# ThibHlln/smartpy

Hardware: AMD Instinct MI355X
Metric: MC sample-timesteps/sec/GPU; 1e5 LHS x hourly 10-yr forcing (higher is better)
Workload: dtype f64

## Files before the change

smartpy_amd/csrc/smart_device.h:

```cpp
#pragma once

#include "smart_matrix_common.h"

#include <hip/hip_runtime.h>

#include <type_traits>

namespace smart {

constexpr int kMaxDiv = 12;
constexpr int kForcingInsane = 1 << 30;

struct KArgs {
    long N, T, W, gap, R, first_len;
    int report_type;
    int np_mean;
    double dt;
    const double *area;
    const double *forcing;
    const double *params;
    long pstride_c;
    const double *extra;
    const double *initial;
    const double *obs;
// ... 843 lines not shown
            else
                body(k, *p1, 0.0, 0.0, std::true_type{});
        }
        if (pass == 0 && n_groups > 0) {
            const long group = (long)kGroup * gap;
            const double2 *__restrict__ p = f0 + (long)n_lead * gap;
            const_f64 pe = obs + n_lead, pw = dev + n_lead;
            double2 cur[kGroup], nxt[kGroup];
            double e_cur[kGroup] = {}, e_nxt[kGroup] = {}, w_cur[kGroup] = {}, w_nxt[kGroup] = {};
#pragma unroll
            for (int j = 0; j < kGroup; ++j) {
                cur[j] = p[j * gap];
                if constexpr (OBS) {
                    e_cur[j] = pe[j];
                    w_cur[j] = pw[j];
                }
            }
#pragma unroll
            for (int j = 0; j < kGroup; ++j) {
                asm volatile("" ::"s"(cur[j].x), "s"(cur[j].y));
                if constexpr (OBS)
                    asm volatile("" ::"s"(e_cur[j]), "s"(w_cur[j]));
            }
            for (int g = 0; g < n_groups; ++g) {
                if (g + 1 < n_groups) {
                    p += group;
                    if constexpr (OBS) {
                        pe += kGroup;
                        pw += kGroup;
                    }
                }
#pragma unroll
                for (int j = 0; j < kGroup; ++j) {
                    nxt[j] = p[j * gap];
                    if constexpr (OBS) {
                        e_nxt[j] = pe[j];
                        w_nxt[j] = pw[j];
                    }
                }
#pragma unroll
                for (int j = 0; j < kGroup; ++j)
                    body(n_lead + g * kGroup + j, cur[j], e_cur[j], w_cur[j], std::false_type{});
#pragma unroll
                for (int j = 0; j < kGroup; ++j) {
                    cur[j] = nxt[j];
                    e_cur[j] = e_nxt[j];
                    w_cur[j] = w_nxt[j];
                }
            }
        }
    }
}

template <class Body>
__device__ __forceinline__ void interval_loop(const double2 *__restrict__ f, long i0, long i1, long gap, Body &&body)
{
    interval_walk<false>(f, nullptr, nullptr, i0, i1, gap, 0,
                         [&](int k, const double2 v, double, double, auto) { body(k, v); });
}

template <class Body>
__device__ __forceinline__ void interval_loop_obs(const double2 *__restrict__ f, const double *obs, const double *dev,
                                                  long i0, long i1, long gap, int lead, Body &&body)
{
    interval_walk<true>(f, obs + i0, dev + i0, i0, i1, gap, lead, body);
}

constexpr int kPollSleep = 100;
constexpr long kDefaultMaxPolls = 1000000;

struct Work {
    long block, c;
    int seg;
};

__device__ __forceinline__ Work claim_work(const KArgs &a, int sliced_kernel)
{
    Work w;
    if (a.n_seg > 1) {
        unsigned t = 0;
        if (threadIdx.x == 0)
            t = __hip_atomic_fetch_add(reinterpret_cast<unsigned *>(a.hdr) + kHdrTicket + sliced_kernel, 1u,
                                       __ATOMIC_RELAXED, __HIP_MEMORY_SCOPE_AGENT);
        t = (unsigned)__builtin_amdgcn_readfirstlane((int)t);
        const long slot = (long)(t % (unsigned long)a.seg_blocks);
        w.seg = (int)(t / (unsigned long)a.seg_blocks);
        w.c = slot / a.n_blocks;
        w.block = slot % a.n_blocks;
    } else {
        w.block = blockIdx.x;
        w.c = blockIdx.y;
        w.seg = 0;
    }
    return w;
}

__device__ __forceinline__ bool wait_for_slice(const KArgs &a, long slot, int seg)
{
    int *flag = a.seg_flag + slot;
    long polls = 0;
    int v;
    while ((v = __hip_atomic_load(flag, __ATOMIC_RELAXED, __HIP_MEMORY_SCOPE_AGENT)) > -seg && v < seg) {
        __builtin_amdgcn_s_sleep(kPollSleep);
        if (++polls > a.max_polls) {
            raise_status(a, kStatusSliceTimeout);
            return false;
        }
    }
    __builtin_amdgcn_fence(__ATOMIC_ACQUIRE, "agent");
    return v >= seg;
}

__device__ __forceinline__ void publish_slice(const KArgs &a, long slot, int seg, bool good)
{
    asm volatile("s_waitcnt vmcnt(0)" ::: "memory");
    __builtin_amdgcn_fence(__ATOMIC_RELEASE, "agent");
    asm volatile("s_waitcnt vmcnt(0)" ::: "memory");
    if (threadIdx.x == 0)
        __hip_atomic_store(a.seg_flag + slot, good ? seg + 1 : -(seg + 1), __ATOMIC_RELAXED, __HIP_MEMORY_SCOPE_AGENT);
}

constexpr int kReportMean = 0, kReportLast = 1, kReportEvery = 2;

template <class Model, int FORCING, int REPORT = kReportMean>
__device__ __forceinline__ void run_ensemble_merged(const KArgs &a, const double2 *__restrict__ forcing,
                                                    const double *__restrict__ obs_all,
                                                    const double *__restrict__ ws_all, long block, long catchment,
                                                    int seg, int fflags)
{
    constexpr bool piecewise = FORCING != kForcingVarying;
    constexpr bool runs = FORCING == kForcingRuns;
    static_assert(REPORT == kReportMean || (!Model::kSplit && !runs), "raw / every-step reports: merged model, no runs");
    static_assert(REPORT != kReportEvery || !piecewise, "a report every step is a step loop");
    static_assert(Model::kStateFields <= kSegPend, "the model's states end in front of the other hand-over fields");
    const LaneCtx x = lane_ctx(a, block, catchment);
    const long slot = catchment * a.n_blocks + block;
    Model m;
    init_model(a, x, m);
    const long gap = a.gap;
    const long run_len = runs ? run_length(a, fflags) : gap;
    if constexpr (piecewise)
        m.setup_intervals(REPORT == kReportLast ? run_len - 1 : run_len);
    const double2 *__restrict__ f = forcing + x.c * a.T;

    int fits = 0;
    unsigned not_quick = ~0u;
    if constexpr (piecewise && Model::kWetAsm) {
        m.note_capacity();
        const bool fits_b = m.over_mask == 0;
        fits = __builtin_amdgcn_readfirstlane((int)fits_b);
        not_quick = 0u - (unsigned)__builtin_amdgcn_readfirstlane((int)!(fits_b && !(fflags & kForcingInsane)));
        asm("" : "+s"(fits), "+s"(not_quick));
    }
    auto no_bits = [](double x, unsigned unless = 0) {
        unsigned long long b = __builtin_bit_cast(unsigned long long, x) | unless;
        asm("" : "+s"(b));
        return b == 0;
    };
    auto interval = [&](const double2 v, double &acc, double &num, double &den) {
        if constexpr (piecewise && Model::kWetAsm) {
            if (no_bits(v.x, not_quick)) {
                if (no_bits(v.y)) {
                    m.calm_interval(run_len, acc);
                } else {
                    m.dry_interval(-v.y, run_len, acc);
                }
                return;
            }
        }
        const double ex = m.excess(v.x, v.y);
        if (ex < 0.0) {
            m.dry_interval(ex, run_len, acc);
        } else {
            if constexpr (piecewise && Model::kWetAsm)
                m.wet_interval(ex, run_len, acc, num, den, fits);
            else
                m.wet_interval(ex, run_len, acc, num, den);
        }
    };

    [[maybe_unused]] auto interval_last = [&](const double2 v, double &qo, double &qg, double &qi) {
        if constexpr (piecewise && REPORT == kReportLast && Model::kWetAsm) {
            double sink = 0.0, n0 = 0.0, n1 = 0.0;
            if (no_bits(v.x, not_quick)) {
                if (no_bits(v.y)) {
                    m.calm_interval(gap - 1, sink);
                    m.last_step_flows(qo, qg, qi);
                    m.calm_interval(1, sink);
                } else {
                    m.dry_interval_last(-v.y, gap, qo, qg, qi);
                }
                return;
            }
            const double ex = m.excess(v.x, v.y);
            if (ex < 0.0) {
                m.dry_interval_last(ex, gap, qo, qg, qi);
            } else {
                m.wet_interval(ex, gap - 1, sink, n0, n1, fits);
                m.last_step_flows(qo, qg, qi);
                m.wet_interval(ex, 1, sink, n0, n1, fits);
            }
        }
    };

    const long n_warm = a.W / gap, n_all = n_warm + a.R;
    const long g0 = n_all * seg / a.n_seg, g1 = n_all * (seg + 1) / a.n_seg;
    const long wa = g0 < n_warm ? g0 : n_warm, wb = g1 < n_warm ? g1 : n_warm;
    const long ra = g0 > n_warm ? g0 - n_warm : 0, rb = g1 > n_warm ? g1 - n_warm : 0;
    const bool last = seg == a.n_seg - 1;

    Reporter rep;
    rep.init(a, x, obs_all, ws_all);
    [[maybe_unused]] const double *__restrict__ obs_c = obs_all ? obs_all + x.c * a.R : nullptr;
    [[maybe_unused]] const double *__restrict__ dev_c = ws_all ? ws_all + x.c * (kWsHead + a.R) + kWsHead : nullptr;
    [[maybe_unused]] const uint2 *codes_c = a.codes ? a.codes + x.c * code_chunks(a.T) : nullptr;
    [[maybe_unused]] const double2 *f_asm = reinterpret_cast<const double2 *>(a.forcing) + x.c * a.T;
    double num = 0.0, den = 0.0, q_out_total = 0.0;
    [[maybe_unused]] double num_raw = 0.0, den_raw = 0.0;
    double *hand = a.seg_state + (slot * kSegFields) * kWave + x.lane;
    if (seg > 0) {
        if (!wait_for_slice(a, slot, seg)) {
            const double nan = quiet_nan();
            if (a.discharge && x.live)
                for (long r = ra; r < rb; ++r)
                    a.discharge[(x.c * a.R + r) * a.ld + x.n] = nan;
            if (last) {
                if (x.live) {
                    a.gw[x.c * a.N + x.n] = nan;
                    if (a.objfn)
                        for (int i = 0; i < 8; ++i)
                            a.objfn[(x.c * a.N + x.n) * 8 + i] = nan;
                    if (a.final_vars)
                        for (int i = 0; i < 19; ++i)
                            a.final_vars[(x.c * a.N + x.n) * 19 + i] = nan;
                }
            } else {
                publish_slice(a, slot, seg, false);
            }
            return;
        }
        m.load_state(hand, kWave);
        if constexpr (REPORT == kReportLast) {
            num_raw = hand[kSegOutflows * kWave];
            den_raw = hand[kSegDenRaw * kWave];
        } else {
            q_out_total = hand[kSegOutflows * kWave];
        }
        rep.A = hand[kSegA * kWave];
        rep.B = hand[kSegB * kWave];
        rep.C1 = hand[kSegC1 * kWave];
        rep.C2 = hand[kSegC2 * kWave];
        rep.C3 = hand[kSegC3 * kWave];
        rep.shift = hand[kSegShift * kWave];
    }

    double *const park = Model::kSplit ? a.final_vars + (x.c * a.N + x.n) * 19 : nullptr;
    auto park_state = [&]() {
        if constexpr (Model::kSplit) {
            m.save_state(park, 1);
            if constexpr (!piecewise)
                park[15] = m.pend;
        }
    };

    double s0 = 0.0, s1 = 0.0, s2 = 0.0;
    const double inv_gap = 1.0 / (double)gap;
    const bool starts_run = ra == 0 && (rb > 0 || last);
    constexpr bool deferring = !piecewise;
    [[maybe_unused]] const bool first_slice = ra == 0;
    [[maybe_unused]] int store = __builtin_amdgcn_readfirstlane((int)(a.discharge != nullptr));
    asm("" : "+s"(store));
    [[maybe_unused]] const int k_park = Model::kSplit && ra <= a.R - 1 && a.R - 1 < rb ? (int)(a.R - 1 - ra) : -1;
    if constexpr (piecewise)
        rep.begin_rows(a, x, ra);
    if constexpr (runs) {
        const long per = gap / run_len;
        interval_loop(f, wa * per, wb * per, run_len, [&](int, const double2 v) { interval(v, s0, s1, s2); });
        if (starts_run)
            m.begin_run();
        long j = 0, r = ra;
        double acc = 0.0;
        rep.prime(a, ra);
        interval_loop(f, ra * per, rb * per, run_len, [&](int, const double2 v) {
            if (Model::kSplit && j == 0 && r == a.R - 1)
                park_state();
            interval(v, acc, num, den);
            if (++j == per) {
                rep.emit_ahead(a, x, r, acc * inv_gap);
                q_out_total += acc;
                acc = 0.0;
                j = 0;
                ++r;
            }
        });
    } else if constexpr (piecewise && REPORT == kReportLast) {
        interval_loop(f, wa, wb, gap, [&](int, const double2 v) { interval_last(v, s0, s1, s2); });
        if (starts_run)
            m.begin_run();
        if (rep.want_obj) {
            interval_loop_obs(f, rep.obs, rep.ws + kWsHead, ra, rb, gap, first_slice ? 1 : 0,
                              [&](int k, const double2 v, const double e, const double w, auto lead_tag) {
                                  double qo, qg, qi;
                                  interval_last(v, qo, qg, qi);
                                  rep.template emit_interval<true, decltype(lead_tag)::value, false>(
                                      store, a.ld, first_slice && k == 0, qo, e, w);
                                  num_raw += qg;
                                  den_raw += qi;
                              });
        } else {
            interval_loop(f, ra, rb, gap, [&](int, const double2 v) {
                double qo, qg, qi;
                interval_last(v, qo, qg, qi);
                rep.template emit_interval<false, false, true>(store, a.ld, false, qo, 0.0, 0.0);
                num_raw += qg;
                den_raw += qi;
            });
        }
    } else if constexpr (piecewise) {
        interval_loop(f, wa, wb, gap, [&](int, const double2 v) { interval(v, s0, s1, s2); });
        if (starts_run)
            m.begin_run();
        if (rep.want_obj) {
            interval_loop_obs(f, rep.obs, rep.ws + kWsHead, ra, rb, gap, first_slice ? 1 : 0,
                              [&](int k, const double2 v, const double e, const double w, auto lead_tag) {
                                  if (Model::kSplit && k == k_park)
                                      park_state();
                                  double acc = 0.0;
                                  interval(v, acc, num, den);
                                  rep.template emit_interval<true, decltype(lead_tag)::value, false>(
                                      store, a.ld, first_slice && k == 0, acc * inv_gap, e, w);
                                  q_out_total += acc;
                              });
        } else {
            interval_loop(f, ra, rb, gap, [&](int k, const double2 v) {
                if (Model::kSplit && k == k_park)
                    park_state();
                double acc = 0.0;
                interval(v, acc, num, den);
                rep.template emit_interval<false, false, true>(store, a.ld, false, acc * inv_gap, 0.0, 0.0);
                q_out_total += acc;
            });
        }
    } else {
        m.begin_lazy(seg > 0 ? hand[kSegPend * kWave] : 0.0);
        long k = 0, r = ra;
        (void)k;
        double acc = 0.0;
        auto report = [&]() __attribute__((always_inline)) {
            auto emit = [&](const double val) __attribute__((always_inline)) {
                rep.emit(a, x, r, val);
                rep.next_row(a);
            };
            if constexpr (REPORT == kReportMean) {
// ... 244 lines not shown
```

smartpy_amd/csrc/smart_fast_arms.h:

```cpp
#pragma once

#define SMART_A_ALIGN8 ".p2align 3\n\t"
#define SMART_A_ALIGN8_ODD ".p2align 3\n\ts_nop 0\n\t"
#define SMART_A_ROUTE                                                                                                  \
    "v_mul_f64 %[t0], %[cg], %[yg]\n\t"                                                                                \
    "v_fma_f64 %[t0], %[cf], %[yf], %[t0]\n\t"                                                                         \
    "v_fma_f64 %[t0], %[cs], %[ys], %[t0]\n\t"                                                                         \
    "v_add_f64 %[acc], %[acc], %[riv]\n\t"                                                                             \
    "v_fma_f64 %[riv], %[riv], %[oma], %[t0]\n\t"
#define SMART_A_ROUTE_LAST                                                                                             \
    "v_mul_f64 %[qg], %[cg], %[yg]\n\t"                                                                                \
    "v_fma_f64 %[qi], %[cf], %[yf], %[qg]\n\t"                                                                         \
    "v_fma_f64 %[qi], %[cs], %[ys], %[qi]\n\t"                                                                         \
    "v_mov_b64_e64 %[acc], %[riv]\n\t"                                                                                 \
    "v_fma_f64 %[riv], %[riv], %[oma], %[qi]\n\t"
#define SMART_A_CASCADE                                                                                                \
    "v_add_f64 %[l0], %[pend], -%[l0]\n\t"                                                                             \
    "v_mul_f64 %[t0], %[pc], %[l0]\n\t"                                                                                \
    "v_max_f64 %[t0], %[t0], 0\n\t"                                                                                    \
    "v_cmp_lt_f64 vcc, 0, %[t0]\n\t"                                                                                   \
    "s_cbranch_vccz 2f\n\t"                                                                                            \
    "v_add_f64 %[l1], %[t0], -%[l1]\n\t"                                                                               \
    "v_mul_f64 %[t0], %[pc], %[l1]\n\t"                                                                                \
    "v_max_f64 %[t0], %[t0], 0\n\t"                                                                                    \
// ... 320 lines not shown
    "91:\n\t" SMART_P_NINE("0", route, "s[36:37]", "s[38:39]", "s[40:41]", "s[42:43]", SMART_P_TAIL_A0, deep,          \
                           calm_split, zeros, drain, rain_split, dry_split)                                            \
        SMART_P_NINE("1", route, "s[44:45]", "s[46:47]", "s[48:49]", "s[50:51]", tail_b0, deep, calm_split, zeros,     \
                     drain, rain_split, dry_split)                                                                     \
            SMART_P_NINE("2", route, "s[52:53]", "s[54:55]", "s[56:57]", "s[58:59]", SMART_P_TAIL_A1, deep,            \
                         calm_split, zeros, drain, rain_split, dry_split)                                              \
                SMART_P_NINE("3", route, "s[60:61]", "s[62:63]", "s[64:65]", "s[66:67]", SMART_P_TAIL_B1, deep,        \
                             calm_split, zeros, drain, rain_split, dry_split)                                          \
                    SMART_P_QUADS("4", "0", "1", route, "s[38:39]", "s[42:43]", "s[46:47]", "s[50:51]", tail_b0, deep, \
                                  calm_split, dry_split)                                                               \
                        SMART_P_QUADS("4", "2", "3", route, "s[54:55]", "s[58:59]", "s[62:63]", "s[66:67]",            \
                                      SMART_P_TAIL_B1, deep, calm_split, dry_split) ".p2align 3\n\t" block94             \
    "95:\n\t" report SMART_P_NEXT_INTERVAL("s[52:67]", "s[70:71]", "s68") "99:\n\t"
#define SMART_A_PAIRS_STRETCH(route, report, deep, calm_split, zeros, drain, rain_split, dry_split)                    \
    SMART_A_PAIRS_STRETCH_X(route, report, SMART_P_ENTRY_EVEN, SMART_P_TAIL_B0, "", deep, calm_split, zeros, drain,    \
                            rain_split, dry_split)
#define SMART_A_PAIRS_STRETCH_ODD(route, report, deep, calm_split, zeros, drain, rain_split, dry_split)                \
    SMART_A_PAIRS_STRETCH_X(route, report, SMART_P_ENTRY_ODD, SMART_P_TAIL_B0_ODD, SMART_P_REPORT94(report), deep,     \
                            calm_split, zeros, drain, rain_split, dry_split)
#define SMART_P_CLOBBERS                                                                                               \
    "s52", "s53", "s54", "s55", "s56", "s57", "s58", "s59", "s60", "s61", "s62", "s63", "s64", "s65", "s66", "s67",    \
        "s70", "s71", "s72", "s73", "s74", "s76", "s77", "s78", "s79", "vcc", "scc"
#define SMART_S_CLOBBERS                                                                                               \
    "s36", "s37", "s38", "s39", "s40", "s41", "s42", "s43", "s44", "s45", "s46", "s47", "s48", "s49", "s50", "s51",    \
        "s68", "s69", "s75", "s80", "s81", "s82", "s83", "s84", "s85", SMART_P_CLOBBERS

#define SMART_E_STORE "global_store_dwordx2 %[row], %[acc], off" SMART_STORE_MOD "\n\tv_lshl_add_u64 %[row], %[ld], 3, %[row]\n\t"
#define SMART_E_MOMENTS(e, w, whi) SMART_R_MOMENTS("%[acc]", e, w, whi)
#define SMART_E_SUM "v_add_f64 %[qtot], %[qtot], %[acc]\n\t"
#define SMART_E_C_N(rep, id) SMART_P_ARM_C_N(SMART_A_ROUTE_LAST, id, "", "") rep
#define SMART_E_C_Q(rep) SMART_P_ARM_C_Q(SMART_A_ROUTE_LAST, "", "") rep
#define SMART_E_C_F(rep) SMART_P_ARM_C_F(SMART_A_ROUTE_LAST, "", "") rep
#define SMART_E_D(pe, rep) SMART_A_DRY(SMART_A_ROUTE_LAST, pe, "") rep
#define SMART_E_R(rn, pe, id, rep) "s_nop 0\n\t" SMART_P_ARM_R(SMART_A_ROUTE_LAST, rn, pe, id, "", "", "", "") "s_nop 0\n\t" rep
#define SMART_E_R_Q(rn, pe, rep) "s_nop 0\n\t" SMART_P_ARM_R_Q(SMART_A_ROUTE_LAST, rn, pe, "", "", "", "") "s_nop 0\n\t" rep
#define SMART_E_R_F(rn, pe, rep) "s_nop 0\n\t" SMART_P_ARM_R_F(SMART_A_ROUTE_LAST, rn, pe, "", "", "", "") "s_nop 0\n\t" rep
#define SMART_E_BLOCK(pos, k, body) ".org 91b+(" pos "*9+" k ")*" SMART_P_STR(SMART_E_STRIDE) "\n\t" body
#define SMART_E_NINE(pos, rx, px, r0, ry, py, r1, tail)                                                                \
    SMART_E_BLOCK(pos, "0", SMART_E_C_N(r0, "0") SMART_E_C_Q(r1) tail SMART_P_OOL(SMART_A_CASC_CALM_OOL("0")))         \
    SMART_E_BLOCK(pos, "1", SMART_E_C_N(r0, "0") SMART_E_D(py, r1) tail SMART_P_OOL(SMART_A_CASC_CALM_OOL("0")))       \
    SMART_E_BLOCK(pos, "2", SMART_E_C_N(r0, "0") SMART_E_R_Q(ry, py, r1) tail SMART_P_OOL(SMART_A_CASC_CALM_OOL("0"))) \
    SMART_E_BLOCK(pos, "3", SMART_E_D(px, r0) SMART_E_C_F(r1) tail)                                                    \
    SMART_E_BLOCK(pos, "4", SMART_E_D(px, r0) SMART_E_D(py, r1) tail)                                                  \
    SMART_E_BLOCK(pos, "5", SMART_E_D(px, r0) SMART_E_R_F(ry, py, r1) tail)                                            \
    SMART_E_BLOCK(pos, "6", SMART_E_R(rx, px, "0", r0) SMART_E_C_N(r1, "1")                                            \
                                tail SMART_P_OOL(SMART_A_CASC_RAIN_OOL("0")) SMART_P_OOL(SMART_A_CASC_CALM_OOL("1")))  \
    SMART_E_BLOCK(pos, "7", SMART_E_R(rx, px, "0", r0) SMART_E_D(py, r1) tail SMART_P_OOL(SMART_A_CASC_RAIN_OOL("0"))) \
    SMART_E_BLOCK(pos, "8", SMART_E_R(rx, px, "0", r0) SMART_E_R(ry, py, "1", r1)                                      \
                                tail SMART_P_OOL(SMART_A_CASC_RAIN_OOL("0")) SMART_P_OOL(SMART_A_CASC_RAIN_OOL("1")))
#define SMART_E_REQUEST(p, c)                                                                                          \
    "s_add_u32 s73, s73, 64\n\t"                                                                                       \
    "s_load_dwordx16 " p ", %[sp], s73\n\t"                                                                            \
    "s_add_u32 s74, s74, 4\n\t"                                                                                        \
    "s_load_dword " c ", %[cp], s74\n\t"
#define SMART_E_TAIL_P0 "s_waitcnt lgkmcnt(0)\n\t" SMART_E_REQUEST("s[36:51]", "s68") SMART_P_JUMP("s70")
#define SMART_E_TAIL_P1                                                                                                \
    "s_waitcnt lgkmcnt(0)\n\t"                                                                                         \
    "s_add_u32 s72, s72, 1\n\t"                                                                                        \
    "s_cbranch_scc1 99f\n\t" SMART_E_REQUEST("s[52:67]", "s70") SMART_P_JUMP("s68")
#define SMART_E_REP(store, mom, e, w, whi) store mom(e, w, whi) SMART_E_SUM
#define SMART_E_NOMOM(e, w, whi) ""
#define SMART_A_EVERY_STREAM(store, mom)                                                                               \
    "s_getpc_b64 s[78:79]\n\t"                                                                                         \
    "90:\n\t"                                                                                                          \
    "s_add_u32 s78, s78, 91f-90b\n\t"                                                                                  \
    "s_addc_u32 s79, s79, 0\n\t"                                                                                       \
    "s_mov_b32 s77, s79\n\t"                                                                                           \
    "s_load_dwordx16 s[36:51], %[sp], 0x0\n\t"                                                                         \
    "s_load_dword s68, %[cp], 0x0\n\t"                                                                                 \
    "s_mov_b32 s73, 64\n\t"                                                                                            \
    "s_load_dwordx16 s[52:67], %[sp], s73\n\t"                                                                         \
    "s_mov_b32 s74, 4\n\t"                                                                                             \
    "s_load_dword s70, %[cp], s74\n\t"                                                                                 \
    "s_sub_u32 s72, 0, %[quads]\n\t"                                                                                   \
    "s_waitcnt lgkmcnt(0)\n\t" SMART_P_JUMP("s68") ".p2align 6\n\t"                                                    \
    "91:\n\t" SMART_E_NINE("0", "s[36:37]", "s[38:39]", SMART_E_REP(store, mom, "s[40:41]", "s[42:43]", "s43"),        \
                           "s[44:45]", "s[46:47]", SMART_E_REP(store, mom, "s[48:49]", "s[50:51]", "s51"),             \
                           SMART_E_TAIL_P0)                                                                            \
        SMART_E_NINE("1", "s[52:53]", "s[54:55]", SMART_E_REP(store, mom, "s[56:57]", "s[58:59]", "s59"), "s[60:61]",  \
                     "s[62:63]", SMART_E_REP(store, mom, "s[64:65]", "s[66:67]", "s67"), SMART_E_TAIL_P1)              \
            ".p2align 3\n\t"                                                                                           \
            "99:\n\t"
#define SMART_E_CLOBBERS                                                                                               \
    "s36", "s37", "s38", "s39", "s40", "s41", "s42", "s43", "s44", "s45", "s46", "s47", "s48", "s49", "s50", "s51",    \
        "s68", SMART_P_CLOBBERS

#define SMART_G_ARM1(arm, rep) arm rep
#define SMART_G_NINE(pos, v, route, rx, px, r0, ry, py, r1, tail)                                                      \
    SMART_E_BLOCK(pos, v "*9+0", SMART_P_ARM_C_N(route, "0", "", "") r0 SMART_P_ARM_C_Q(route, "", "") r1              \
                                     tail SMART_P_OOL(SMART_A_CASC_CALM_OOL("0")))                                     \
    SMART_E_BLOCK(pos, v "*9+1", SMART_P_ARM_C_N(route, "0", "", "") r0 SMART_A_DRY(route, py, "") r1                  \
                                     tail SMART_P_OOL(SMART_A_CASC_CALM_OOL("0")))                                     \
    SMART_E_BLOCK(pos, v "*9+2", SMART_P_ARM_C_N(route, "0", "", "") r0 "s_nop 0\n\t" SMART_P_ARM_R_Q(                 \
        route, ry, py, "", "", "", "") "s_nop 0\n\t" r1 tail SMART_P_OOL(SMART_A_CASC_CALM_OOL("0")))                  \
    SMART_E_BLOCK(pos, v "*9+3", SMART_A_DRY(route, px, "") r0 SMART_P_ARM_C_F(route, "", "") r1 tail)                 \
    SMART_E_BLOCK(pos, v "*9+4", SMART_A_DRY(route, px, "") r0 SMART_A_DRY(route, py, "") r1 tail)                     \
    SMART_E_BLOCK(pos, v "*9+5", SMART_A_DRY(route, px, "") r0 "s_nop 0\n\t" SMART_P_ARM_R_F(                          \
        route, ry, py, "", "", "", "") "s_nop 0\n\t" r1 tail)                                                          \
    SMART_E_BLOCK(pos, v "*9+6", "s_nop 0\n\t" SMART_P_ARM_R(route, rx, px, "0", "", "", "", "") "s_nop 0\n\t" r0      \
                                     SMART_P_ARM_C_N(route, "1", "", "") r1                                            \
                                         tail SMART_P_OOL(SMART_A_CASC_RAIN_OOL("0"))                                  \
                                             SMART_P_OOL(SMART_A_CASC_CALM_OOL("1")))                                  \
    SMART_E_BLOCK(pos, v "*9+7", "s_nop 0\n\t" SMART_P_ARM_R(route, rx, px, "0", "", "", "", "") "s_nop 0\n\t" r0      \
                                     SMART_A_DRY(route, py, "") r1 tail SMART_P_OOL(SMART_A_CASC_RAIN_OOL("0")))       \
    SMART_E_BLOCK(pos, v "*9+8", "s_nop 0\n\t" SMART_P_ARM_R(route, rx, px, "0", "", "", "", "") "s_nop 0\n\t" r0      \
                                     "s_nop 0\n\t" SMART_P_ARM_R(route, ry, py, "1", "", "", "", "") "s_nop 0\n\t" r1  \
                                         tail SMART_P_OOL(SMART_A_CASC_RAIN_OOL("0"))                                  \
                                             SMART_P_OOL(SMART_A_CASC_RAIN_OOL("1")))
#define SMART_G_REP(value, after, e, w, whi) SMART_P_REPORT_X(value, after, e, w, whi) "s_nop 0\n\t"
#define SMART_G_THREE(pos, route, value, after, rx, px, e0, w0, h0, ry, py, e1, w1, h1, tail)                          \
    SMART_G_NINE(pos, "0", route, rx, px, "", ry, py, "", tail)                                                        \
    SMART_G_NINE(pos, "1", route, rx, px, SMART_G_REP(value, after, e0, w0, h0), ry, py, "", tail)                     \
    SMART_G_NINE(pos, "2", route, rx, px, "", ry, py, SMART_G_REP(value, after, e1, w1, h1), tail)
#define SMART_A_GAP_STREAM(route, value, after)                                                                        \
    "s_getpc_b64 s[78:79]\n\t"                                                                                         \
    "90:\n\t"                                                                                                          \
    "s_add_u32 s78, s78, 91f-90b\n\t"                                                                                  \
    "s_addc_u32 s79, s79, 0\n\t"                                                                                       \
    "s_mov_b32 s77, s79\n\t"                                                                                           \
    "s_load_dwordx16 s[36:51], %[sp], 0x0\n\t"                                                                         \
    "s_load_dword s68, %[cp], 0x0\n\t"                                                                                 \
    "s_mov_b32 s73, 64\n\t"                                                                                            \
    "s_load_dwordx16 s[52:67], %[sp], s73\n\t"                                                                         \
    "s_mov_b32 s74, 4\n\t"                                                                                             \
    "s_load_dword s70, %[cp], s74\n\t"                                                                                 \
    "s_sub_u32 s72, 0, %[quads]\n\t"                                                                                   \
    "s_mov_b32 s85, %[r0]\n\t"                                                                                         \
    "s_waitcnt lgkmcnt(0)\n\t" SMART_P_JUMP("s68") ".p2align 6\n\t"                                                    \
    "91:\n\t" SMART_G_THREE("0", route, value, after, "s[36:37]", "s[38:39]", "s[40:41]", "s[42:43]", "s43",           \
                            "s[44:45]", "s[46:47]", "s[48:49]", "s[50:51]", "s51", SMART_E_TAIL_P0)                    \
        SMART_G_THREE("3", route, value, after, "s[52:53]", "s[54:55]", "s[56:57]", "s[58:59]", "s59", "s[60:61]",     \
                      "s[62:63]", "s[64:65]", "s[66:67]", "s67", SMART_E_TAIL_P1) ".p2align 3\n\t"                     \
                                                                                   "99:\n\t"

#define SMART_A_WET_HEAD SMART_A_ROUTE "v_fma_f64 %[xf], -%[eh], %[tot], %[ex]\n\t" SMART_A_FILL1("l0", "xf")
#define SMART_A_WET_FILL_TAIL                                                                                          \
    SMART_A_FILL1("l1", "t1") SMART_A_FILL1("l2", "t1") SMART_A_FILL1("l3", "t1") SMART_A_FILL1("l4", "t1")            \
        SMART_A_FILL1("l5", "t1") "v_mul_f64 %[xs], %[eh], %[tot]\n\t"                                                 \
                                  "v_fma_f64 %[xf], -%[pd], %[t1], %[xf]\n\t"                                          \
                                  "v_fma_f64 %[xs], %[pd], %[t1], %[xs]\n\t"
#define SMART_A_WET_REST                                                                                               \
    SMART_A_LEAKS_("s1", "p2", "p3", "") "v_add_f64 %[t1], %[tot], -%[ai]\n\t"                                                            \
                    "v_add_f64 %[xf], %[xf], %[t1]\n\t" SMART_A_TOT_XG                                                 \
                    "v_fma_f64 %[ys], %[ys], %[ds], %[xs]\n\t"                                                         \
                    "v_fma_f64 %[yf], %[yf], %[df], %[xf]\n\t"                                                         \
                    "v_fma_f64 %[yg], %[yg], %[dg], %[xg]\n\t"                                                         \
                    "v_add_f64 %[xgs], %[xgs], %[xg]\n\t"
#define SMART_A_WET_STEP SMART_A_WET_HEAD SMART_A_WET_FILL_TAIL SMART_A_WET_REST
#define SMART_A_WET_ABSORBED(fix)                                                                                      \
    SMART_A_WET_HEAD "v_cmp_nle_f64 vcc, %[t1], 0\n\t"                                                                 \
                     "s_cbranch_vccnz " fix "f\n\t"                                                                    \
                     "v_mul_f64 %[xs], %[eh], %[tot]\n\t" SMART_A_WET_REST
#define SMART_A_WET_FULL(fix) SMART_A_WET_HEAD fix ":\n\t" SMART_A_WET_FILL_TAIL SMART_A_WET_REST
#define SMART_A_WET_GROUPS                                                                                             \
    "s_lshr_b32 %[cnt], %[n], 2\n\t"                                                                                  \
    "s_sub_u32 %[cnt], 0, %[cnt]\n\t"                                                                                  \
    "s_cbranch_scc0 9f\n\t"
#define SMART_A_WET_INTERVAL                                                                                           \
    SMART_A_ALIGN8 "s_cmp_eq_u32 %[ok], 0\n\t"                                                                         \
    "s_cbranch_scc1 40f\n\t"                                                                                           \
    "s_and_b32 %[cnt], %[n], 3\n\t"                                                                                  \
    "s_cbranch_scc0 20f\n\t"                                                                                           \
    "s_sub_u32 %[cnt], 0, %[cnt]\n\t"                                                                                  \
    "5:\n\t" SMART_A_WET_ABSORBED("7") "s_add_u32 %[cnt], %[cnt], 1\n\t"                                               \
    "s_cbranch_scc0 5b\n\t"                                                                                            \
    "20:\n\t" SMART_A_WET_GROUPS "25:\n\t" SMART_A_WET_ABSORBED("71") "s_nop 0\n\t" SMART_A_WET_ABSORBED("72")         \
    "s_nop 0\n\t" SMART_A_WET_ABSORBED("73") "s_nop 0\n\t" SMART_A_WET_ABSORBED("74")                        \
    "s_add_u32 %[cnt], %[cnt], 1\n\t"                                                                                  \
    "s_cbranch_scc0 25b\n\t"                                                                                           \
    "s_branch 9f\n\t"                                                                                                  \
    "40:\n\t"                                                                                                          \
    "s_and_b32 %[cnt], %[n], 3\n\t"                                                                                  \
    "s_cbranch_scc0 30f\n\t"                                                                                           \
    "s_sub_u32 %[cnt], 0, %[cnt]\n\t"                                                                                  \
    "6:\n\t" SMART_A_WET_FULL("7") "s_add_u32 %[cnt], %[cnt], 1\n\t"                                                   \
    "s_cbranch_scc0 6b\n\t"                                                                                            \
    "30:\n\t" SMART_A_WET_GROUPS "s_nop 0\n\t"                                                                         \
    "31:\n\t" SMART_A_WET_FULL("71") SMART_A_WET_FULL("72") SMART_A_WET_FULL("73") SMART_A_WET_FULL("74")              \
    "s_add_u32 %[cnt], %[cnt], 1\n\t"                                                                                  \
    "s_cbranch_scc0 31b\n\t"                                                                                           \
    "9:\n\t"
#define SMART_A_CALM_STEP                                                                                              \
    SMART_A_ROUTE SMART_A_LEAKS_("s1", "p2", "p3", "") "v_add_f64 %[xf], %[tot], -%[ai]\n\t" SMART_A_TOT_XG            \
    "v_fma_f64 %[ys], %[ys], %[ds], 0\n\t"                                                                             \
    "v_fma_f64 %[yf], %[yf], %[df], %[xf]\n\t"                                                                         \
    "v_fma_f64 %[yg], %[yg], %[dg], %[xg]\n\t"                                                                         \
    "v_add_f64 %[xgs], %[xgs], %[xg]\n\t"
#define SMART_A_CALM_INTERVAL                                                                                          \
    SMART_A_ALIGN8 "s_add_i32 %[cnt], %[n], 1\n\t"                                                                                    \
    "s_lshr_b32 %[cnt], %[cnt], 1\n\t"                                                                                 \
    "s_bitcmp1_b32 %[n], 0\n\t"                                                                                        \
    "s_cbranch_scc1 6f\n\t"                                                                                            \
    "5:\n\t" SMART_A_CALM_STEP "6:\n\t" SMART_A_CALM_STEP "s_add_i32 %[cnt], %[cnt], -1\n\t"                           \
    "s_cmp_lg_u32 %[cnt], 0\n\t"                                                                                       \
    "s_cbranch_scc1 5b\n\t"
```

smartpy_amd/csrc/smart_fast_model.h:

```cpp
#pragma once

#include "smart_device.h"
#include "smart_fast_arms.h"

namespace smart {

template <bool STIFF, bool GUARD, bool MERGE = false, bool EXITS = true, bool SPLIT = false>
struct FastModel {
    static_assert(!(MERGE && STIFF), "the clamps of structure.py:429-450 act on each reservoir separately");
    static_assert(MERGE || !SPLIT, "SPLIT refines the merged form");
    static constexpr bool kExactDivide = false;
    static constexpr bool kSplit = SPLIT;

    double pT, pC, pD, hz, sz, z;
    double dec_s, dec_f, dec_g, cq_s, cq_f, cq_g;
    double a_r, inv_a_r;
    double a_s, a_f, a_g;
    double car_s, car_f, car_g, om_ar;
    double k_s, k_f, k_g, k_r, mm_to_m3;
    double l0, l1, l2, l3, l4, l5;
    double u_ove, u_dra, u_int, u_sgw, u_dgw, u_riv;
    double q_out, q_in, q_gw;

    __device__ void setup(double area, double dt, const double *p)
// ... 186 lines not shown
    }

    __device__ static void sum_then_fma_in_place(double &sum, double &y, double a, double x)
    {
        asm("v_add_f64 %0, %0, %1\n\tv_fma_f64 %1, %1, %2, %3" : "+v"(sum), "+v"(y) : "v"(a), "v"(x));
    }


    __device__ __forceinline__ void wet_lanes(double ex)
    {
        if (kLeakBalance) {
            double tot = layer_sum();
            wet_balance(ex, ex * hz, tot);
            return;
        }
        const double tot = layer_sum();
        const double hp = hz * tot;
        const double s1 = sz * tot;
        const double of = hp * ex;
        ex = fma(-hp, ex, ex);
        fill(l0, ex, z);
        if (excess_left(ex)) {
            fill(l1, ex, z);
            fill(l2, ex, z);
            fill(l3, ex, z);
            fill(l4, ex, z);
            fill(l5, ex, z);
        }
        const double df = pD * ex;
        double inf = ex - df;
        double sh = 0.0, dp = 0.0;
        const double p2 = s1 * s1, p3 = p2 * s1, p4 = p2 * p2, p5 = p4 * s1, p6 = p3 * p3;
        leak(l0, s1, s1, p6, inf, sh, dp);
        leak(l1, p2, s1 * 0.5, p5, inf, sh, dp);
        leak(l2, p3, s1 * (1.0 / 3.0), p4, inf, sh, dp);
        leak(l3, p4, s1 * 0.25, p3, inf, sh, dp);
        leak(l4, p5, s1 * 0.2, p2, inf, sh, dp);
        leak(l5, p6, s1 * (1.0 / 6.0), s1, inf, sh, dp);
        if (MERGE) {
            const double xg = sh + dp;
            u_ove = fma(u_ove, dec_s, of + df);
            u_int = fma(u_int, dec_f, inf);
            u_sgw = fma(u_sgw, dec_g, xg);
            if (kBalanceSums)
                xg_sum += xg;
        } else {
            u_ove = clamp(fma(u_ove, dec_s, of * cq_s));
            u_dra = clamp(fma(u_dra, dec_s, df * cq_s));
            u_int = clamp(fma(u_int, dec_f, inf * cq_f));
            u_sgw = clamp(fma(u_sgw, dec_g, sh * cq_g));
            u_dgw = clamp(fma(u_dgw, dec_g, dp * cq_g));
        }
    }

    static constexpr bool kLeakBalance = MERGE && !GUARD;
    static_assert(kLeakBalance || !SPLIT, "SPLIT is implemented in wet_balance()");

    static constexpr bool kExits = EXITS;

    __device__ __forceinline__ double deep_leak(double s1, double p2, double p3, double p4, double p5, double p6) const
    {
        return fma(l5, s1, fma(l4, p2, fma(l3, p3, fma(l2, p4, fma(l1, p5, l0 * p6)))));
    }

    __device__ __forceinline__ static double opaque_zero()
    {
        double x;
        asm volatile("v_mov_b64 %0, 0" : "=v"(x));
        return x;
    }

    __device__ static void fill3(double &l, double &ex, double z)
    {
        const double t = l + ex;
        l = fmin(t, z);
        ex = t - l;
    }

    __device__ __forceinline__ void wet_balance(const double ex, const double e_h, double &tot)
    {
        const double s1 = sz * tot;
        const double ex_in = fma(-e_h, tot, ex);
        double rem = ex_in;
        fill3(l0, rem, z);
        if (!kExits || excess_left(rem)) {
            fill3(l1, rem, z);
            if (!kExits || excess_left(rem)) {
                fill3(l2, rem, z);
                fill3(l3, rem, z);
                fill3(l4, rem, z);
                fill3(l5, rem, z);
            }
        }
        const double p2 = s1 * s1, p3 = p2 * s1, p4 = p2 * p2, p5 = p4 * s1, p6 = p3 * p3;
        l0 = fma(-l0, s1, l0);
        l1 = fma(-l1, p2, l1);
        l2 = fma(-l2, p3, l2);
        l3 = fma(-l3, p4, l3);
        l4 = fma(-l4, p5, l4);
        l5 = fma(-l5, p6, l5);
        const double after_int = layer_sum();
        l0 = fma(-l0, s1, l0);
        l1 = fma(-l1, s1 * 0.5, l1);
        l2 = fma(-l2, s1 * (1.0 / 3.0), l2);
        l3 = fma(-l3, s1 * 0.25, l3);
        l4 = fma(-l4, s1 * 0.2, l4);
        l5 = fma(-l5, s1 * (1.0 / 6.0), l5);
        const double deep = SPLIT ? deep_leak(s1, p2, p3, p4, p5, p6) : 0.0;
        l0 = fma(-l0, p6, l0);
        l1 = fma(-l1, p5, l1);
        l2 = fma(-l2, p4, l2);
        l3 = fma(-l3, p3, l3);
        l4 = fma(-l4, p2, l4);
        l5 = fma(-l5, s1, l5);
        const double inf = (tot - after_int) + fma(-pD, rem, ex_in);
        fma_in_place(u_ove, dec_s, fma(pD, rem, e_h * tot));
        fma_in_place(u_int, dec_f, inf);
        const double upper = (l0 + l1) + (l2 + l3), lower = l4 + l5;
        asm("v_add_f64 %0, %1, %2" : "+v"(tot) : "v"(upper), "v"(lower));
        const double xg = after_int - tot;
        fma_in_place(u_sgw, dec_g, xg);
        if (SPLIT) {
            fma_in_place(u_dra, dec_s, pD * rem);
            fma_in_place(u_dgw, dec_g, deep);
        }
        if (kBalanceSums)
            xg_sum += xg;
    }

#ifndef SMART_WET_ASM
#define SMART_WET_ASM 1
#endif
    static constexpr bool kWetAsm = SMART_WET_ASM && kLeakBalance && !kExits && !SPLIT && !STIFF;

    __device__ __forceinline__ void calm_interval(long n, double &acc)
    {
        static_assert(kWetAsm, "calm_interval() is the asm loop of the straight-line merged kernels");
        double tot = layer_sum();
        double t0, t1, xf, xg, w_s1, w_p2, w_p3, w_p4, w_p5, w_p6, w_ai;
        int cnt;
        asm volatile(SMART_A_CALM_INTERVAL
                     : [l0] "+v"(l0), [l1] "+v"(l1), [l2] "+v"(l2), [l3] "+v"(l3), [l4] "+v"(l4), [l5] "+v"(l5),
                       [ys] "+v"(u_ove), [yf] "+v"(u_int), [yg] "+v"(u_sgw), [riv] "+v"(u_riv), [acc] "+v"(acc),
                       [tot] "+v"(tot), [xgs] "+v"(xg_sum), [t0] "=&v"(t0), [t1] "=&v"(t1), [xf] "=&v"(xf),
                       [xg] "=&v"(xg), [s1] "=&v"(w_s1), [p2] "=&v"(w_p2), [p3] "=&v"(w_p3), [p4] "=&v"(w_p4),
                       [p5] "=&v"(w_p5), [p6] "=&v"(w_p6), [ai] "=&v"(w_ai), [cnt] "=&s"(cnt)
                     : [cs] "v"(car_s), [cf] "v"(car_f), [cg] "v"(car_g), [oma] "v"(om_ar), [ds] "v"(dec_s),
                       [df] "v"(dec_f), [dg] "v"(dec_g), [sz] "v"(sz), [k3] "s"(-(1.0 / 3.0)), [k5] "s"(-0.2),
                       [k6] "s"(-(1.0 / 6.0)), [n] "s"((int)n)
                     : "scc");
    }

    __device__ __forceinline__ void wet_interval(double ex, long n, double &acc, double &num, double &den,
                                                 const int fits = 0)
    {
        if constexpr (kWetAsm) {
            const double e_h = ex * hz;
            double tot = layer_sum();
            double t0, t1, xs, xf, xg, w_s1, w_p2, w_p3, w_p4, w_p5, w_p6, w_ai;
            int cnt;
            asm volatile(SMART_A_WET_INTERVAL
                         : [l0] "+v"(l0), [l1] "+v"(l1), [l2] "+v"(l2), [l3] "+v"(l3), [l4] "+v"(l4), [l5] "+v"(l5),
                           [ys] "+v"(u_ove), [yf] "+v"(u_int), [yg] "+v"(u_sgw), [riv] "+v"(u_riv), [acc] "+v"(acc),
                           [tot] "+v"(tot), [xgs] "+v"(xg_sum), [t0] "=&v"(t0), [t1] "=&v"(t1), [xs] "=&v"(xs),
                           [xf] "=&v"(xf), [xg] "=&v"(xg), [s1] "=&v"(w_s1), [p2] "=&v"(w_p2), [p3] "=&v"(w_p3),
                           [p4] "=&v"(w_p4), [p5] "=&v"(w_p5), [p6] "=&v"(w_p6), [ai] "=&v"(w_ai), [cnt] "=&s"(cnt)
                         : [cs] "v"(car_s), [cf] "v"(car_f), [cg] "v"(car_g), [oma] "v"(om_ar), [ds] "v"(dec_s),
                           [df] "v"(dec_f), [dg] "v"(dec_g), [sz] "v"(sz), [z] "v"(z), [pd] "v"(pD), [ex] "v"(ex),
                           [eh] "v"(e_h), [k3] "s"(-(1.0 / 3.0)), [k5] "s"(-0.2), [k6] "s"(-(1.0 / 6.0)),
                           [n] "s"((int)n), [ok] "s"(fits)
                         : "scc", "vcc");
        } else if (kLeakBalance) {
            const double e_h = ex * hz;
            double tot = layer_sum();
#pragma unroll 1
            for (long k = 0; k < n; ++k) {
                route_and_sum(acc, num, den);
                wet_balance(ex, e_h, tot);
            }
        } else {
            for (long k = 0; k < n; ++k) {
                route_and_sum(acc, num, den);
                wet_lanes(ex);
            }
        }
    }

    __device__ __forceinline__ void dry_lanes(double ex)
    {
        double d = -ex;
        dry(l0, d, pC);
        auto handed_down = [](double x) { return GUARD ? x != 0.0 : x > 0.0; };
        if (__builtin_amdgcn_ballot_w64(handed_down(d)) != 0) {
            dry(l1, d, pC);
            if (__builtin_amdgcn_ballot_w64(handed_down(d)) != 0) {
                dry(l2, d, pC);
                dry(l3, d, pC);
                dry(l4, d, pC);
                dry(l5, d, pC);
            }
        }
        u_ove = clamp(u_ove * dec_s);
        u_int = clamp(u_int * dec_f);
        u_sgw = clamp(u_sgw * dec_g);
        if (!MERGE || SPLIT) {
            u_dra = clamp(u_dra * dec_s);
            u_dgw = clamp(u_dgw * dec_g);
        }
    }

    __device__ __forceinline__ void route_and_sum(double &acc, double &num, double &den)
    {
        double q_r = u_riv;
        double u_new;
        if (MERGE && !STIFF && kBalanceSums) {
            q_out = u_riv;
            q_gw = cq_g * u_sgw;
            q_in = fma(cq_s, u_ove, fma(cq_f, u_int, q_gw));
            const double y = fma(car_s, u_ove, fma(car_f, u_int, car_g * u_sgw));
            if (kExits) {
                sum_then_fma_in_place(acc, u_riv, om_ar, y);
            } else {
                acc += u_riv;
                fma_in_place(u_riv, om_ar, y);
            }
            return;
        }
        if (MERGE) {
            u_new = u_riv;
            fma_in_place(u_new, om_ar, fma(car_s, u_ove, fma(car_f, u_int, car_g * u_sgw)));
            q_gw = cq_g * u_sgw;
            q_in = fma(cq_s, u_ove, fma(cq_f, u_int, q_gw));
        } else {
            q_gw = u_sgw + u_dgw;
            q_in = ((u_ove + u_dra) + u_int) + q_gw;
            u_new = fma(q_in - u_riv, a_r, u_riv);
        }
        if (STIFF) {
            if (u_new < 0.0) {
                q_r = 0.95 * fma(u_riv, inv_a_r, q_in);
                u_new = fma(q_in - q_r, a_r, u_riv);
            }
        }
        u_riv = u_new;
        q_out = q_r;
        acc += q_r;
        if (!kBalanceSums) {
            num += q_gw;
            den += q_in;
        }
    }

    static constexpr int kStateFields = 15;

    __device__ void save_state(double *p, int stride) const
    {
        const double v[kStateFields] = {l0, l1, l2, l3, l4, l5, u_ove, u_int, u_sgw, u_riv, g0, r0, xg_sum, u_dra, u_dgw};
#pragma unroll
        for (int i = 0; i < (SPLIT ? 15 : 13); ++i)
            p[i * stride] = v[i];
    }

    __device__ void load_state(const double *p, int stride)
    {
        double v[kStateFields] = {};
#pragma unroll
        for (int i = 0; i < (SPLIT ? 15 : 13); ++i)
            v[i] = p[i * stride];
        l0 = v[0], l1 = v[1], l2 = v[2], l3 = v[3], l4 = v[4], l5 = v[5];
        u_ove = v[6], u_int = v[7], u_sgw = v[8], u_riv = v[9];
        g0 = v[10], r0 = v[11], xg_sum = v[12];
        u_dra = v[13], u_dgw = v[14];
        note_capacity();
    }

    static constexpr bool kBalanceSums = MERGE;
    double g0, r0, xg_sum;

    __device__ void begin_run()
    {
        g0 = u_sgw;
        r0 = u_riv;
        xg_sum = 0.0;
    }

    __device__ void balance_sums(double q_out_total, double &num, double &den) const
    {
        num = cq_g * (xg_sum + (g0 - u_sgw)) / (1.0 - dec_g);
        den = fma(u_riv - r0, inv_a_r, q_out_total);
    }

    __device__ void step(double , double , double ex, double &acc, double &num, double &den)
    {
        if (ex >= 0.0) {
            route_and_sum(acc, num, den);
            wet_lanes(ex);
        } else {
            route_and_sum(acc, num, den);
            dry_lanes(ex);
        }
    }

    __device__ void step(double r, double e, double ex, double &acc, double &num, double &den, StepGeneric)
    {
        step(r, e, ex, acc, num, den);
    }

    __device__ void step(double, double, double ex, double &acc, double &num, double &den, StepAllWet)
    {
        route_and_sum(acc, num, den);
        wet_lanes(ex);
    }

    double pend, tot_c;
    bool zero_ok;
    unsigned long long pend_mask;

    __device__ void begin_lazy(double pending)
    {
        pend = pending;
        pend_mask = __builtin_amdgcn_ballot_w64(pending > 0.0);
        tot_c = layer_sum();
        note_capacity();
// ... 458 lines not shown
```

smartpy_amd/csrc/smart_fast_runs.hip:

```cpp
#include "smart_fast_entry.h"

namespace smart {

SMART_FAST_KERNEL(smart_fast_runs_exits) { merged_kernel<FastModel<false, false, true, true>, kForcingRuns>(a, forcing, obs, ws); }

SMART_FAST_KERNEL(smart_fast_runs) { merged_kernel<FastModel<false, false, true, false>, kForcingRuns>(a, forcing, obs, ws); }

SMART_FAST_KERNEL(smart_fast_runs_states)
{
    merged_kernel<FastModel<false, false, true, true, true>, kForcingRuns>(a, forcing, obs, ws);
}

}
```

Measured before the change: 899.8 billion.

## Run wet intervals under explicit exec mask and reorder divergent dry/calm branches

The wet interval asm now sets the exec mask itself via s_and_saveexec from a ballot of wet lanes, and computes e_h and the layer sum inside the asm. The control flow is reshaped so that the wet, dry and calm paths are taken as separate predicated regions instead of nested branches with an early return, with the aim of cutting divergence overhead. The grouped-by-4 loop now runs before the remainder loop. The main runs kernel also gets a waves_per_eu(2,2) attribute to change register and occupancy tradeoffs. The new structure risks running more paths per interval when lanes mix, and the occupancy pin may cost latency hiding.

```diff
diff --git a/smartpy_amd/csrc/smart_device.h b/smartpy_amd/csrc/smart_device.h
--- a/smartpy_amd/csrc/smart_device.h
+++ b/smartpy_amd/csrc/smart_device.h
@@ -1019,28 +1019,35 @@
         not_quick = 0u - (unsigned)__builtin_amdgcn_readfirstlane((int)!(fits_b && !(fflags & kForcingInsane)));
         asm("" : "+s"(fits), "+s"(not_quick));
     }
-    auto no_bits = [](double x, unsigned unless = 0) {
+    auto bits_of = [](double x, unsigned unless = 0) {
         unsigned long long b = __builtin_bit_cast(unsigned long long, x) | unless;
         asm("" : "+s"(b));
-        return b == 0;
+        return b;
+    };
+    auto same_bits = [](unsigned long long b) {
+        asm("" : "+s"(b));
+        return b;
     };
     auto interval = [&](const double2 v, double &acc, double &num, double &den) {
         if constexpr (piecewise && Model::kWetAsm) {
-            if (no_bits(v.x, not_quick)) {
-                if (no_bits(v.y)) {
+            const unsigned long long rainy = bits_of(v.x, not_quick);
+            if (rainy != 0) {
+                const double ex = m.excess(v.x, v.y);
+                const bool dry = ex < 0.0;
+                m.wet_interval(ex, run_len, acc, num, den, fits, __builtin_amdgcn_ballot_w64(true) & ~__builtin_amdgcn_ballot_w64(dry));
+                if (dry)
+                    m.dry_interval(ex, run_len, acc);
+            }
+            if (same_bits(rainy) == 0) {
+                if (bits_of(v.y) != 0)
+                    m.dry_interval(-v.y, run_len, acc);
+                else
                     m.calm_interval(run_len, acc);
-                } else {
-                    m.dry_interval(-v.y, run_len, acc);
-                }
-                return;
-            }
-        }
-        const double ex = m.excess(v.x, v.y);
-        if (ex < 0.0) {
-            m.dry_interval(ex, run_len, acc);
+            }
         } else {
-            if constexpr (piecewise && Model::kWetAsm)
-                m.wet_interval(ex, run_len, acc, num, den, fits);
+            const double ex = m.excess(v.x, v.y);
+            if (ex < 0.0)
+                m.dry_interval(ex, run_len, acc);
             else
                 m.wet_interval(ex, run_len, acc, num, den);
         }
@@ -1049,23 +1056,25 @@
     [[maybe_unused]] auto interval_last = [&](const double2 v, double &qo, double &qg, double &qi) {
         if constexpr (piecewise && REPORT == kReportLast && Model::kWetAsm) {
             double sink = 0.0, n0 = 0.0, n1 = 0.0;
-            if (no_bits(v.x, not_quick)) {
-                if (no_bits(v.y)) {
+            const unsigned long long rainy = bits_of(v.x, not_quick);
+            if (rainy != 0) {
+                const double ex = m.excess(v.x, v.y);
+                const bool dry = ex < 0.0;
+                const unsigned long long wet = __builtin_amdgcn_ballot_w64(true) & ~__builtin_amdgcn_ballot_w64(dry);
+                m.wet_interval(ex, gap - 1, sink, n0, n1, fits, wet);
+                m.last_step_flows(qo, qg, qi);
+                m.wet_interval(ex, 1, sink, n0, n1, fits, wet);
+                if (dry)
+                    m.dry_interval_last(ex, gap, qo, qg, qi);
+            }
+            if (same_bits(rainy) == 0) {
+                if (bits_of(v.y) != 0) {
+                    m.dry_interval_last(-v.y, gap, qo, qg, qi);
+                } else {
                     m.calm_interval(gap - 1, sink);
                     m.last_step_flows(qo, qg, qi);
                     m.calm_interval(1, sink);
-                } else {
-                    m.dry_interval_last(-v.y, gap, qo, qg, qi);
                 }
-                return;
-            }
-            const double ex = m.excess(v.x, v.y);
-            if (ex < 0.0) {
-                m.dry_interval_last(ex, gap, qo, qg, qi);
-            } else {
-                m.wet_interval(ex, gap - 1, sink, n0, n1, fits);
-                m.last_step_flows(qo, qg, qi);
-                m.wet_interval(ex, 1, sink, n0, n1, fits);
             }
         }
     };
diff --git a/smartpy_amd/csrc/smart_fast_arms.h b/smartpy_amd/csrc/smart_fast_arms.h
--- a/smartpy_amd/csrc/smart_fast_arms.h
+++ b/smartpy_amd/csrc/smart_fast_arms.h
@@ -496,34 +496,35 @@
                      "s_cbranch_vccnz " fix "f\n\t"                                                                    \
                      "v_mul_f64 %[xs], %[eh], %[tot]\n\t" SMART_A_WET_REST
 #define SMART_A_WET_FULL(fix) SMART_A_WET_HEAD fix ":\n\t" SMART_A_WET_FILL_TAIL SMART_A_WET_REST
-#define SMART_A_WET_GROUPS                                                                                             \
-    "s_lshr_b32 %[cnt], %[n], 2\n\t"                                                                                  \
+#define SMART_A_WET_TURNS(none)                                                                                        \
+    "s_lshr_b32 %[cnt], %[n], 2\n\t"                                                                                   \
     "s_sub_u32 %[cnt], 0, %[cnt]\n\t"                                                                                  \
-    "s_cbranch_scc0 9f\n\t"
+    "s_cbranch_scc0 " none "f\n\t"
+#define SMART_A_WET_SINGLES                                                                                            \
+    "s_and_b32 %[cnt], %[n], 3\n\t"                                                                                    \
+    "s_cbranch_scc0 9f\n\t"                                                                                            \
+    "s_sub_u32 %[cnt], 0, %[cnt]\n\t"
 #define SMART_A_WET_INTERVAL                                                                                           \
-    SMART_A_ALIGN8 "s_cmp_eq_u32 %[ok], 0\n\t"                                                                         \
-    "s_cbranch_scc1 40f\n\t"                                                                                           \
-    "s_and_b32 %[cnt], %[n], 3\n\t"                                                                                  \
-    "s_cbranch_scc0 20f\n\t"                                                                                           \
-    "s_sub_u32 %[cnt], 0, %[cnt]\n\t"                                                                                  \
-    "5:\n\t" SMART_A_WET_ABSORBED("7") "s_add_u32 %[cnt], %[cnt], 1\n\t"                                               \
-    "s_cbranch_scc0 5b\n\t"                                                                                            \
-    "20:\n\t" SMART_A_WET_GROUPS "25:\n\t" SMART_A_WET_ABSORBED("71") "s_nop 0\n\t" SMART_A_WET_ABSORBED("72")         \
-    "s_nop 0\n\t" SMART_A_WET_ABSORBED("73") "s_nop 0\n\t" SMART_A_WET_ABSORBED("74")                        \
+    SMART_A_ALIGN8 "s_and_saveexec_b64 %[sv], %[wm]\n\t"                                                               \
+    "s_cbranch_execz 9f\n\t"                                                                                           \
+    "v_mul_f64 %[eh], %[ex], %[hz]\n\t" SMART_A_LSUM("tot") "s_cmp_eq_u32 %[ok], 0\n\t"                                \
+    "s_cbranch_scc1 40f\n\t" SMART_A_WET_TURNS("20")                                                                   \
+    "25:\n\t" SMART_A_WET_ABSORBED("71") "s_nop 0\n\t" SMART_A_WET_ABSORBED("72")                                      \
+    "s_nop 0\n\t" SMART_A_WET_ABSORBED("73") "s_nop 0\n\t" SMART_A_WET_ABSORBED("74")                                  \
     "s_add_u32 %[cnt], %[cnt], 1\n\t"                                                                                  \
     "s_cbranch_scc0 25b\n\t"                                                                                           \
+    "20:\n\t" SMART_A_WET_SINGLES "5:\n\t" SMART_A_WET_ABSORBED("7") "s_add_u32 %[cnt], %[cnt], 1\n\t"                 \
+    "s_cbranch_scc0 5b\n\t"                                                                                            \
     "s_branch 9f\n\t"                                                                                                  \
-    "40:\n\t"                                                                                                          \
-    "s_and_b32 %[cnt], %[n], 3\n\t"                                                                                  \
-    "s_cbranch_scc0 30f\n\t"                                                                                           \
-    "s_sub_u32 %[cnt], 0, %[cnt]\n\t"                                                                                  \
-    "6:\n\t" SMART_A_WET_FULL("7") "s_add_u32 %[cnt], %[cnt], 1\n\t"                                                   \
-    "s_cbranch_scc0 6b\n\t"                                                                                            \
-    "30:\n\t" SMART_A_WET_GROUPS "s_nop 0\n\t"                                                                         \
+    "40:\n\t" SMART_A_WET_TURNS("30")                                                                                  \
     "31:\n\t" SMART_A_WET_FULL("71") SMART_A_WET_FULL("72") SMART_A_WET_FULL("73") SMART_A_WET_FULL("74")              \
     "s_add_u32 %[cnt], %[cnt], 1\n\t"                                                                                  \
     "s_cbranch_scc0 31b\n\t"                                                                                           \
-    "9:\n\t"
+    "30:\n\t" SMART_A_WET_SINGLES "s_nop 0\n\t"                                                                        \
+    "6:\n\t" SMART_A_WET_FULL("7") "s_add_u32 %[cnt], %[cnt], 1\n\t"                                                   \
+    "s_cbranch_scc0 6b\n\t"                                                                                            \
+    "9:\n\t"                                                                                                           \
+    "s_or_b64 exec, exec, %[sv]\n\t"
 #define SMART_A_CALM_STEP                                                                                              \
     SMART_A_ROUTE SMART_A_LEAKS_("s1", "p2", "p3", "") "v_add_f64 %[xf], %[tot], -%[ai]\n\t" SMART_A_TOT_XG            \
     "v_fma_f64 %[ys], %[ys], %[ds], 0\n\t"                                                                             \
diff --git a/smartpy_amd/csrc/smart_fast_model.h b/smartpy_amd/csrc/smart_fast_model.h
--- a/smartpy_amd/csrc/smart_fast_model.h
+++ b/smartpy_amd/csrc/smart_fast_model.h
@@ -362,23 +362,23 @@
     }
 
     __device__ __forceinline__ void wet_interval(double ex, long n, double &acc, double &num, double &den,
-                                                 const int fits = 0)
+                                                 const int fits = 0, const unsigned long long wet = 0)
     {
         if constexpr (kWetAsm) {
-            const double e_h = ex * hz;
-            double tot = layer_sum();
-            double t0, t1, xs, xf, xg, w_s1, w_p2, w_p3, w_p4, w_p5, w_p6, w_ai;
+            double tot, e_h, t0, t1, xs, xf, xg, w_s1, w_p2, w_p3, w_p4, w_p5, w_p6, w_ai;
+            unsigned long long saved;
             int cnt;
             asm volatile(SMART_A_WET_INTERVAL
                          : [l0] "+v"(l0), [l1] "+v"(l1), [l2] "+v"(l2), [l3] "+v"(l3), [l4] "+v"(l4), [l5] "+v"(l5),
                            [ys] "+v"(u_ove), [yf] "+v"(u_int), [yg] "+v"(u_sgw), [riv] "+v"(u_riv), [acc] "+v"(acc),
-                           [tot] "+v"(tot), [xgs] "+v"(xg_sum), [t0] "=&v"(t0), [t1] "=&v"(t1), [xs] "=&v"(xs),
-                           [xf] "=&v"(xf), [xg] "=&v"(xg), [s1] "=&v"(w_s1), [p2] "=&v"(w_p2), [p3] "=&v"(w_p3),
-                           [p4] "=&v"(w_p4), [p5] "=&v"(w_p5), [p6] "=&v"(w_p6), [ai] "=&v"(w_ai), [cnt] "=&s"(cnt)
+                           [xgs] "+v"(xg_sum), [tot] "=&v"(tot), [eh] "=&v"(e_h), [t0] "=&v"(t0), [t1] "=&v"(t1),
+                           [xs] "=&v"(xs), [xf] "=&v"(xf), [xg] "=&v"(xg), [s1] "=&v"(w_s1), [p2] "=&v"(w_p2),
+                           [p3] "=&v"(w_p3), [p4] "=&v"(w_p4), [p5] "=&v"(w_p5), [p6] "=&v"(w_p6), [ai] "=&v"(w_ai),
+                           [cnt] "=&s"(cnt), [sv] "=&s"(saved)
                          : [cs] "v"(car_s), [cf] "v"(car_f), [cg] "v"(car_g), [oma] "v"(om_ar), [ds] "v"(dec_s),
                            [df] "v"(dec_f), [dg] "v"(dec_g), [sz] "v"(sz), [z] "v"(z), [pd] "v"(pD), [ex] "v"(ex),
-                           [eh] "v"(e_h), [k3] "s"(-(1.0 / 3.0)), [k5] "s"(-0.2), [k6] "s"(-(1.0 / 6.0)),
-                           [n] "s"((int)n), [ok] "s"(fits)
+                           [hz] "v"(hz), [k3] "s"(-(1.0 / 3.0)), [k5] "s"(-0.2), [k6] "s"(-(1.0 / 6.0)),
+                           [n] "s"((int)n), [ok] "s"(fits), [wm] "s"(wet)
                          : "scc", "vcc");
         } else if (kLeakBalance) {
             const double e_h = ex * hz;
diff --git a/smartpy_amd/csrc/smart_fast_runs.hip b/smartpy_amd/csrc/smart_fast_runs.hip
--- a/smartpy_amd/csrc/smart_fast_runs.hip
+++ b/smartpy_amd/csrc/smart_fast_runs.hip
@@ -4,7 +4,7 @@
 
 SMART_FAST_KERNEL(smart_fast_runs_exits) { merged_kernel<FastModel<false, false, true, true>, kForcingRuns>(a, forcing, obs, ws); }
 
-SMART_FAST_KERNEL(smart_fast_runs) { merged_kernel<FastModel<false, false, true, false>, kForcingRuns>(a, forcing, obs, ws); }
+__attribute__((amdgpu_waves_per_eu(2, 2))) SMART_FAST_KERNEL(smart_fast_runs) { merged_kernel<FastModel<false, false, true, false>, kForcingRuns>(a, forcing, obs, ws); }
 
 SMART_FAST_KERNEL(smart_fast_runs_states)
 {
```

After: 908.1 billion (median of 4 runs). Within noise of the previous version (+0.9%).
